# tuffy/libdvd-audio

Measured on AMD Instinct MI355X. Metric: decoded PCM Msamples/s (bit-exact) on 6ch/96k/24b MLP, higher is better.
Workload: dtype int32 (int64 accumulate)

## Files before the change

### libdvd-audio_amd/csrc/mlp_ctx.h

```cpp
#pragma once
#include <vector>

#include "hip_ws.h"
#include "mlp_decode.h"
#include "mlp_conceal.h"
#include "mlp_index.h"

using namespace mlp;

constexpr uint32_t EV_RING = 256;
constexpr uint32_t SEQ_ROUND = 1024;

struct DecodeSettings {
    uint32_t lanes_per_seg = 0;
    uint32_t pcm_layout = DVDA_PCM_PLANAR;
    uint32_t chain_form = 0;
    const int32_t *d_init_fir = nullptr;
};

struct ConcealInfo {
    uint32_t valid, status;
    uint64_t rows, frames;
};

struct ConcealState {
    bool on = false;
    dvda_mlp_hip_ctx *child = nullptr;
    DevBuf<ConcealPlan> d_plan;
    DevBuf<uint8_t> d_bytes;
    DevBuf<uint64_t> d_tab;
    DevBuf<int32_t> d_scr[CONCEAL_ROUNDS];
    DevBuf<ConcealOp> d_ops;
    DevBuf<int32_t> d_fir;
    std::vector<std::vector<dvda_mlp_conceal_span>> spans;
    std::vector<ConcealInfo> info;

    ~ConcealState() { dvda_mlp_hip_destroy(child); }
};

struct PresentState {
    uint32_t mode = DVDA_PRESENT_FULL;
    dvda_mlp_hip_ctx *child = nullptr;
    DevBuf<uint8_t> d_bytes;
    uint64_t bound = 0;
    DevBuf<uint32_t> d_info;
    DevBuf<uint32_t> d_size;
    DevBuf<uint32_t> d_sbase;
    DevBuf<uint32_t> d_len;
    DevBuf<uint32_t> d_base;
    DevBuf<uint64_t> d_off64, d_len64;
    Event ev[2];
    bool ev_set = false;
    bool map_valid = false;
    uint32_t h_nseg = 0;
    std::vector<SegRec> h_seg;
    std::vector<uint32_t> h_sbase, h_base, h_info;
    std::vector<StreamRec> h_streams;

    ~PresentState() { dvda_mlp_hip_destroy(child); }
};

struct dvda_mlp_hip_ctx {
    int device;
    uint32_t coop_min_seg;
    uint32_t max_streams, max_segments;
    DevBuf<uint8_t> d_masks;
    DevBuf<uint16_t> d_parts;
    DevBuf<uint32_t> d_tile_count;
    DevBuf<uint32_t> d_tile_base;
    DevBuf<uint64_t> d_cand_off;
    DevBuf<SegRec> d_seg;
    DevBuf<uint32_t> d_seg_frames;
    DevBuf<uint32_t> d_seg_fbase;
    DevBuf<uint32_t> d_seg_status;
    DevBuf<uint32_t> d_seg_rows;
    DevBuf<StreamRec> d_streams;
    uint32_t *d_n_cand;
    DevBuf<uint32_t> d_scan_tmp;
    DevBuf<int32_t> d_iir;
    DevBuf<uint32_t> d_mat;
    DevBuf<unsigned long long> d_dbg;
    DevBuf<int32_t> d_fir;
    DevBuf<uint32_t> d_seg_meta;
    DevBuf<uint32_t> d_yield;
    DevBuf<uint32_t> d_seg_check;
    DevBuf<uint32_t> d_cls;
    DevBuf<uint32_t> d_shape_key;
    DevBuf<uint64_t> d_soff, d_slen;
    DevBuf<uint32_t> d_rank;
    DevBuf<uint32_t> d_sorted_cnt;
    DevBuf<uint32_t> d_sorted_base;
    DevBuf<uint32_t> d_lane_seg;
    DevBuf<DecodeSummary> d_summary;
    DecodeSummary *h_summary;
    Stream st_aux;
    Event ev_fork, ev_join;
    DevBuf<uint32_t> d_seq_list;
    DevBuf<uint4> d_plan;
    DevBuf<uint4> d_scan4_tmp;
    DevBuf<uint32_t> d_def_list;
    DevBuf<uint32_t> d_head_list;
    DevBuf<uint32_t> d_chain_order;
    DevBuf<uint32_t> d_chain_hist;
    DevBuf<int32_t> d_fb;
    uint32_t rsv_segs;
    DevBuf<int32_t> d_res;
    DevBuf<uint32_t> d_brec;
    DevBuf<uint32_t> d_frec;
    uint32_t iir_lanes;
    DevBuf<dvda_pcm_crc_desc> d_crc_desc;
    DevBuf<uint32_t> d_crc_out;
    DevBuf<uint64_t> d_crc_bytes;
    DevBuf<uint32_t> d_crc_work;
    DecodeSettings set;
    const uint8_t *d_bytes;
    uint64_t total_bytes;
    const uint64_t *d_stream_off;
    const uint64_t *d_stream_len;
    uint32_t n_streams;
    uint64_t tiles;
    bool indexed;
    bool small_input;
    bool decoded;
    GraphExec idx_graph;
    const void *idx_key[4];
    uint64_t idx_key_bytes;
    uint32_t idx_key_streams;
    int idx_graph_state;
    Event ev[2 * EV_RING];
    Event ev_end[EV_RING];
    uint64_t ev_count;
    ConcealState cc;
    PresentState pp;

    uint32_t fb_slots() const { return (uint32_t)(d_fb.cap / FB_WORDS); }
    ~dvda_mlp_hip_ctx() { (void)hipHostFree(h_summary); }
};

static WsCaps ws_caps(const dvda_mlp_hip_ctx *c)
{
    WsCaps w;
    w.res = c->d_res.cap;
    w.brec = c->d_brec.cap;
    w.frec = c->d_frec.cap;
    w.fb = c->d_fb.cap;
    w.max_seg = c->max_segments;
    w.max_streams = c->max_streams;
    w.lanes = c->iir_lanes;
    w.pad = 0;
    return w;
}

static inline dvda_mlp_hip_ctx *pp_inner(const dvda_mlp_hip_ctx *c)
{
    return c && c->pp.mode == DVDA_PRESENT_SUBSTREAM0 ? c->pp.child : nullptr;
}

static inline void fill_sync_fields(dvda_mlp_stream_info &o, uint32_t sync)
{
    o.assignment = (sync >> 16) & 0x1F;
    o.substreams = (sync >> 24) & 0xF;
    o.group0_bps = sync & 0xF;
    o.group1_bps = (sync >> 4) & 0xF;
    o.group0_rate = (sync >> 8) & 0xF;
    o.group1_rate = (sync >> 12) & 0xF;
}

static void enqueue_exscan(hipStream_t st, const uint32_t *in, uint32_t *out, uint32_t *tmp, uint32_t n_host,
                           const uint32_t *n_ptr, uint32_t n_cap)
{
    const uint32_t n_max = n_ptr ? n_cap : n_host;
    if (n_max <= 4096) {
        hipLaunchKernelGGL(k_exscan_u32, dim3(1), dim3(1024), 0, st, in, out, n_host, n_ptr, n_cap);
        return;
    }
    const uint32_t blocks = (n_max + 1023) / 1024;
    hipLaunchKernelGGL(k_scan_blocks, dim3(blocks), dim3(1024), 0, st, in, out, tmp, n_host, n_ptr, n_cap);
    hipLaunchKernelGGL(k_exscan_u32, dim3(1), dim3(1024), 0, st, tmp, tmp, blocks, (const uint32_t *)nullptr, blocks);
    hipLaunchKernelGGL(k_scan_add, dim3(blocks), dim3(1024), 0, st, out, tmp, blocks, n_host, n_ptr, n_cap);
}
```

### libdvd-audio_amd/csrc/mlp_hip.hip

```cpp
#include <hip/hip_runtime.h>
#include <math.h>
#include <stdint.h>
#include <stdio.h>
#include <stdlib.h>
#include <string.h>
#include <new>
#include <vector>

#include "../../include/dvda_mlp_hip.h"
#include "mlp_step.h"
#include "mlp_decode.h"
#include "mlp_chain.h"
#include "mlp_chain_small.h"
#include "mlp_check.h"
#include "mlp_coop.h"
#include "mlp_index.h"
#include "mlp_conceal.h"
#include "mlp_present.h"
#include "pcm_unswizzle.h"
#include "wav_pack.h"
#include "pcm_digest.h"

#include "mlp_ctx.h"
#include "mlp_conceal_run.h"
#include "mlp_present_run.h"
#include "mlp_stepper.h"
#include "mlp_tiers.h"
#include "pcm_digest_run.h"

extern "C" int dvda_mlp_hip_bounds_violations(unsigned long long *out4)
{
    if (!out4)
        return DVDA_HIP_EINVAL;
    out4[0] = out4[1] = out4[2] = out4[3] = 0;
#if defined(DVDA_BOUNDS)
    HIP_TRY(hipDeviceSynchronize());
    HIP_TRY(hipMemcpyFromSymbol(out4, HIP_SYMBOL(mlp::g_bounds), 4 * sizeof(unsigned long long)));
    return 1;
#else
    return DVDA_HIP_OK;
#endif
}

extern "C" const char *dvda_mlp_hip_version(void) { return "dvda-mlp-hip 0.1 (gfx950)"; }

extern "C" int dvda_mlp_hip_create(dvda_mlp_hip_ctx **out, int device, uint32_t max_streams,
                                   uint32_t max_segments)
{
    if (!out || max_streams == 0 || max_segments == 0)
        return DVDA_HIP_EINVAL;
    int ndev = 0;
    if (hipGetDeviceCount(&ndev) != hipSuccess || ndev <= 0 || device < 0 || device >= ndev) {
        fprintf(stderr, "dvda_mlp_hip: no usable HIP device (count=%d, requested=%d)\n", ndev, device);
        return DVDA_HIP_ENODEV;
    }
    HIP_TRY(hipSetDevice(device));
    dvda_mlp_hip_ctx *c = new (std::nothrow) dvda_mlp_hip_ctx();
    if (!c)
        return DVDA_HIP_ENOMEM;
    c->device = device;
    {
        int cus = 0;
        if (hipDeviceGetAttribute(&cus, hipDeviceAttributeMultiprocessorCount, device) != hipSuccess || cus <= 0)
            cus = 256;
        c->coop_min_seg = (uint32_t)cus * 4u * 64u * 7u / 4u;
        if (const char *e = getenv("DVDA_COOP_MIN_SEG"))
            c->coop_min_seg = (uint32_t)strtoul(e, nullptr, 10);
    }
    c->max_streams = max_streams;
    c->max_segments = max_segments;
    c->idx_graph_state = getenv("DVDA_INDEX_GRAPH") && atoi(getenv("DVDA_INDEX_GRAPH")) == 0 ? -1 : 0;
    const size_t ns = (size_t)max_segments, nt = (size_t)max_streams;
    c->iir_lanes = (uint32_t)(((2 * ns + DEC_THREADS - 1) / DEC_THREADS) * DEC_THREADS);
    const size_t nl = c->iir_lanes;
    hipError_t e = hipSuccess;
    auto alloc = [&](auto &buf, size_t n) {
        if (e == hipSuccess)
            e = buf.alloc(n);
    };
    alloc(c->d_cand_off, ns);
    alloc(c->d_seg, ns + 4);
    alloc(c->d_seg_frames, ns + 1);
    alloc(c->d_seg_fbase, ns + 5);
    alloc(c->d_seg_status, ns + 4);
    alloc(c->d_seg_rows, ns);
    alloc(c->d_streams, nt);
    alloc(c->d_iir, nl * MAXCH * 16);
    alloc(c->d_mat, nl * MAXMAT * 5);
    alloc(c->d_dbg, 32);
    alloc(c->d_fir, nl * 6 * 8);
    alloc(c->d_seg_meta, nl + 4);
    alloc(c->d_yield, ns);
    alloc(c->d_seg_check, 2 * ns);
    alloc(c->d_cls, 4);
    alloc(c->d_shape_key, nt);
    alloc(c->d_soff, nt);
    alloc(c->d_slen, nt);
    alloc(c->d_rank, nt);
    alloc(c->d_sorted_cnt, nt + 1);
    alloc(c->d_sorted_base, nt + 1);
    alloc(c->d_lane_seg, ns);
    alloc(c->d_summary, 1 + SUMMARY_PARTS);
    alloc(c->d_seq_list, nt);
    alloc(c->d_plan, ns + 5);
    alloc(c->d_scan4_tmp, ns / 1024 + 4);
    alloc(c->d_def_list, ns);
    alloc(c->d_head_list, ns);
    alloc(c->d_chain_order, ns);
    alloc(c->d_chain_hist, 2 * CHAIN_BUCKETS);
    if (e == hipSuccess)
        e = hipHostMalloc((void **)&c->h_summary, sizeof(DecodeSummary), hipHostMallocDefault);
    if (e == hipSuccess)
        e = hipStreamCreateWithFlags(c->st_aux.put(), hipStreamNonBlocking);
    if (e == hipSuccess)
        e = hipEventCreateWithFlags(c->ev_fork.put(), hipEventDisableTiming);
    if (e == hipSuccess)
        e = hipEventCreateWithFlags(c->ev_join.put(), hipEventDisableTiming);
    if (e == hipSuccess)
        e = hipMemset(c->d_dbg, 0, 32 * sizeof(unsigned long long));
    if (e == hipSuccess)
        e = hipMemset(c->d_seg_meta, 0, nl * sizeof(uint32_t));
    for (uint32_t i = 0; e == hipSuccess && i < 2 * EV_RING; i++)
        e = hipEventCreate(c->ev[i].put());
    for (uint32_t i = 0; e == hipSuccess && i < EV_RING; i++)
        e = hipEventCreate(c->ev_end[i].put());
    if (e != hipSuccess) {
        fprintf(stderr, "dvda_mlp_hip: workspace allocation failed: %s\n", hipGetErrorString(e));
        delete c;
        return DVDA_HIP_ENOMEM;
    }
    *out = c;
    return DVDA_HIP_OK;
}

extern "C" void dvda_mlp_hip_destroy(dvda_mlp_hip_ctx *c)
{
    if (!c)
        return;
    (void)hipSetDevice(c->device);
#if defined(DVDA_BOUNDS)
    if (getenv("DVDA_BOUNDS_REPORT")) {
        unsigned long long v[4] = {0, 0, 0, 0};
        (void)dvda_mlp_hip_bounds_violations(v);
        fprintf(stderr, "dvda_mlp_hip: bounds violations: %llu", v[0]);
        if (v[0])
            fprintf(stderr, " (first: tag %llu index %llu capacity %llu)", v[1], v[2], v[3]);
        fprintf(stderr, "\n");
    }
#endif
    delete c;
}

static int ensure_byte_ws(dvda_mlp_hip_ctx *c, uint64_t total_bytes)
{
    const uint64_t chunks = (total_bytes + 15) / 16 + 4;
    const uint64_t tiles = (chunks + IDX_TILE_CHUNKS - 1) / IDX_TILE_CHUNKS;
    auto grow_pair = [](auto &a, uint64_t na, auto &b, uint64_t nb) {
        if (na <= a.cap)
            return DVDA_HIP_OK;
        a.release();
        b.release();
        if (a.alloc(na) == hipSuccess && b.alloc(nb) == hipSuccess)
            return DVDA_HIP_OK;
        a.release();
        return DVDA_HIP_ENOMEM;
    };
    int rc = grow_pair(c->d_masks, chunks, c->d_parts, chunks + 72);
    if (rc)
        return rc;
    uint64_t most = tiles > c->max_segments ? tiles : c->max_segments;
    if (c->max_streams > most)
        most = c->max_streams;
    if ((rc = c->d_scan_tmp.grow_exact((most + 1023) / 1024 + 2)) != 0)
        return rc;
    return grow_pair(c->d_tile_count, tiles + 1, c->d_tile_base, tiles + 1);
}

__global__ void k_init_streams(StreamRec *s, uint32_t n, uint32_t *seg_status, uint32_t *seg_rows, uint32_t *yield_req,
                               uint32_t *seg_meta, uint32_t n_seg, uint32_t *cls, uint32_t *summary_words)
{
    const uint32_t i = blockIdx.x * blockDim.x + threadIdx.x;
    if (i < 4)
        cls[i] = 0;
    if (i < (1 + SUMMARY_PARTS) * sizeof(DecodeSummary) / sizeof(uint32_t))
        summary_words[i] = 0;
    if (i < n_seg) {
        seg_status[i] = 0;
        seg_rows[i] = 0;
        yield_req[i] = 0;
        seg_meta[2 * (size_t)i] = seg_meta[2 * (size_t)i + 1] = 0;
    }
    if (i < n) {
        StreamRec r;
        r.first_seg = 0xFFFFFFFFu;
        r.n_seg = 0;
        r.sync = 0;
        r.status = 0;
        r.frames = 0;
        r.consumed = 0;
        r.rows = 0;
        s[i] = r;
    }
}

__global__ void k_reset_segments(uint32_t *seg_status, uint32_t *seg_rows, uint32_t *yield_req, uint32_t *seg_meta,
                                 uint32_t n_seg)
{
    const uint32_t i = blockIdx.x * blockDim.x + threadIdx.x;
    if (i < n_seg) {
        seg_status[i] = 0;
        seg_rows[i] = 0;
        yield_req[i] = 0;
        seg_meta[2 * (size_t)i] = seg_meta[2 * (size_t)i + 1] = 0;
    }
}

__device__ __forceinline__ void check_ranges_block(const uint64_t *__restrict__ off, const uint64_t *__restrict__ len,
                                                   uint32_t n, uint64_t total_bytes, uint64_t *__restrict__ soff,
                                                   uint64_t *__restrict__ slen, StreamRec *__restrict__ streams,
                                                   unsigned long long *s_max)
{
    const uint32_t per = (n + 1023u) / 1024u;
    const uint32_t lo = threadIdx.x * per, hi = lo + per < n ? lo + per : n;
    auto end_of = [&](uint32_t i) {
        const uint64_t o = off[i], l = len[i];
        return (o <= total_bytes && l <= total_bytes - o && (o & 15u) == 0) ? o + l : 0;
    };
    unsigned long long m = 0;
    for (uint32_t i = lo; i < hi; i++) {
        const unsigned long long e = end_of(i);
        m = e > m ? e : m;
    }
    s_max[threadIdx.x] = m;
    __syncthreads();
    for (uint32_t d = 1; d < 1024u; d <<= 1) {
        const unsigned long long v = threadIdx.x >= d ? s_max[threadIdx.x - d] : 0ull;
        __syncthreads();
        if (v > s_max[threadIdx.x])
            s_max[threadIdx.x] = v;
        __syncthreads();
    }
    unsigned long long run = threadIdx.x ? s_max[threadIdx.x - 1] : 0ull;
    for (uint32_t i = lo; i < hi; i++) {
        const uint64_t o = off[i], l = len[i];
        const bool ok = (o & 15u) == 0 && o <= total_bytes && l <= total_bytes - o && o >= run;
        const uint64_t so = ok ? o : run;
        soff[i] = so < total_bytes ? so : total_bytes;
        slen[i] = ok ? l : 0;
        if (!ok)
            streams[i].status = ST_ENVELOPE | (1u << 16);
        const unsigned long long e = end_of(i);
        run = e > run ? e : run;
    }
}

__global__ __launch_bounds__(1024) void k_check_ranges(const uint64_t *__restrict__ off, const uint64_t *__restrict__ len,
                                                       uint32_t n, uint64_t total_bytes, uint64_t *__restrict__ soff,
                                                       uint64_t *__restrict__ slen, StreamRec *__restrict__ streams)
{
    __shared__ unsigned long long s_max[1024];
    check_ranges_block(off, len, n, total_bytes, soff, slen, streams, s_max);
}

constexpr uint64_t SMALL_INPUT_BYTES = 4096u * 1024u;

static void enqueue_index(dvda_mlp_hip_ctx *c, hipStream_t st, const uint8_t *d_bytes, uint64_t total_bytes,
                          const uint64_t *d_stream_off, const uint64_t *d_stream_len, uint32_t n_streams)
{
    const uint64_t tiles = c->tiles;
    const uint32_t ms = c->max_segments;
    {
        uint32_t n_init = n_streams > ms ? n_streams : ms;
        if (n_init < 1024)
            n_init = 1024;
        hipLaunchKernelGGL(k_init_streams, dim3((n_init + 255) / 256), dim3(256), 0, st, c->d_streams,
                           n_streams, c->d_seg_status, c->d_seg_rows, c->d_yield, c->d_seg_meta, ms, c->d_cls,
                           reinterpret_cast<uint32_t *>(c->d_summary.p));
        hipLaunchKernelGGL(k_check_ranges, dim3(1), dim3(1024), 0, st, d_stream_off, d_stream_len, n_streams, total_bytes,
                           c->d_soff, c->d_slen, c->d_streams);
        d_stream_off = c->d_soff;
        d_stream_len = c->d_slen;
    }
    hipLaunchKernelGGL(k_sync_mask, dim3((unsigned)tiles), dim3(IDX_THREADS), 0, st, d_bytes,
                       total_bytes, c->d_masks, c->d_tile_count, c->d_parts);
    enqueue_exscan(st, c->d_tile_count, c->d_tile_base, c->d_scan_tmp, (uint32_t)tiles, nullptr, (uint32_t)tiles);
    hipLaunchKernelGGL(k_sync_scatter, dim3((unsigned)tiles), dim3(IDX_THREADS), 0, st, c->d_masks,
                       total_bytes, c->d_tile_base, c->d_cand_off, ms);
    hipLaunchKernelGGL(k_chase, dim3((ms + 255) / 256), dim3(256), 0, st, d_bytes, d_stream_off,
                       d_stream_len, n_streams, c->d_cand_off, c->d_n_cand, ms, c->d_seg,
                       c->d_seg_frames, c->d_streams, c->d_cls);
    hipLaunchKernelGGL(k_mark_dead, dim3((ms + 255) / 256), dim3(256), 0, st, d_stream_off, d_stream_len,
                       c->d_n_cand, ms, c->d_seg, c->d_seg_frames, c->d_streams);
    enqueue_exscan(st, c->d_seg_frames, c->d_seg_fbase, c->d_scan_tmp, 0u, c->d_n_cand, ms);
    const bool pack = !(total_bytes <= SMALL_INPUT_BYTES);
    hipLaunchKernelGGL(k_link, dim3((ms + 255) / 256), dim3(256), 0, st, d_stream_off, d_stream_len,
                       c->d_n_cand, ms, c->d_seg, c->d_seg_fbase, c->d_streams, n_streams, c->d_shape_key,
                       c->d_cls + (pack ? 2 : 3));
    hipStream_t sp = st;
    bool forked = false;
    if (pack && st != nullptr && c->st_aux && hipEventRecord(c->ev_fork, st) == hipSuccess &&
        hipStreamWaitEvent(c->st_aux, c->ev_fork, 0) == hipSuccess) {
        sp = c->st_aux;
        forked = true;
    }
    if (pack) {
    hipLaunchKernelGGL(k_stream_rank, dim3((n_streams + 255) / 256), dim3(256), 0, sp, c->d_shape_key, c->d_streams,
                       n_streams, c->d_rank, c->d_sorted_cnt, c->d_cls + 2);
    enqueue_exscan(sp, c->d_sorted_cnt, c->d_sorted_base, c->d_scan_tmp, n_streams, nullptr, n_streams);
    (void)hipMemsetAsync(c->d_lane_seg, 0xFF, (size_t)ms * sizeof(uint32_t), sp);
    hipLaunchKernelGGL(k_lane_perm, dim3((ms + 255) / 256), dim3(256), 0, sp, c->d_seg, c->d_streams, c->d_n_cand, ms,
                       c->d_rank, c->d_sorted_base, c->d_cls + 2, c->d_lane_seg);
    }
    hipLaunchKernelGGL(k_au_check, dim3((unsigned)(((uint64_t)ms * CHK_GROUP + CHK_THREADS - 1) / CHK_THREADS)),
                       dim3(CHK_THREADS), 0, st, d_bytes, c->d_parts, c->d_seg, c->d_n_cand, ms, c->d_streams, c->d_seg_check);
    if (forked) {
        (void)hipEventRecord(c->ev_join, sp);
        (void)hipStreamWaitEvent(st, c->ev_join, 0);
    }
}

static int index_source(dvda_mlp_hip_ctx *c, const uint8_t *d_bytes, uint64_t total_bytes,
                        const uint64_t *d_stream_off, const uint64_t *d_stream_len, uint32_t n_streams, void *stream_)
{
    if (!c || !d_bytes || !d_stream_off || !d_stream_len || n_streams == 0 || total_bytes == 0)
        return DVDA_HIP_EINVAL;
    if (n_streams > c->max_streams)
        return DVDA_HIP_ECAPACITY;
    if (((uintptr_t)d_bytes & 15) != 0)
        return DVDA_HIP_EINVAL;
    hipStream_t st = (hipStream_t)stream_;
    HIP_TRY(hipSetDevice(c->device));
    c->cc.spans.clear();
    c->cc.info.clear();
    int rc = ensure_byte_ws(c, total_bytes);
    if (rc)
        return rc;
    c->d_bytes = d_bytes;
    c->total_bytes = total_bytes;
    c->d_stream_off = d_stream_off;
    c->d_stream_len = d_stream_len;
    c->n_streams = n_streams;
    const uint64_t chunks = (total_bytes + 15) / 16;
    const uint64_t tiles = (chunks + IDX_TILE_CHUNKS - 1) / IDX_TILE_CHUNKS;
    c->tiles = tiles;
    c->d_n_cand = c->d_tile_base + tiles;

    c->small_input = total_bytes <= SMALL_INPUT_BYTES;
    const bool same = c->idx_graph_state > 0 && c->idx_key[0] == d_bytes && c->idx_key[1] == d_stream_off &&
                      c->idx_key[2] == d_stream_len && c->idx_key[3] == (const void *)st &&
                      c->idx_key_bytes == total_bytes && c->idx_key_streams == n_streams;
    if (c->idx_graph_state == 2 && same) {
        if (hipGraphLaunch(c->idx_graph, st) == hipSuccess) {
            c->indexed = true;
            c->decoded = false;
            return DVDA_HIP_OK;
        }
        (void)hipGetLastError();
        c->idx_graph_state = -1;
    } else if (c->idx_graph_state == 1 && same && st != nullptr) {
        hipGraph_t g = nullptr;
        bool ok = hipStreamBeginCapture(st, hipStreamCaptureModeThreadLocal) == hipSuccess;
        if (ok) {
            enqueue_index(c, st, d_bytes, total_bytes, d_stream_off, d_stream_len, n_streams);
            ok = hipStreamEndCapture(st, &g) == hipSuccess && g != nullptr;
        }
        if (ok) {
            ok = hipGraphInstantiate(c->idx_graph.put(), g, nullptr, nullptr, 0) == hipSuccess;
        }
        if (g)
            (void)hipGraphDestroy(g);
        if (ok && hipGraphLaunch(c->idx_graph, st) == hipSuccess) {
            c->idx_graph_state = 2;
            c->indexed = true;
            c->decoded = false;
            return DVDA_HIP_OK;
        }
        (void)hipGetLastError();
        c->idx_graph_state = -1;
    } else if (c->idx_graph_state >= 0) {
        c->idx_key[0] = d_bytes;
        c->idx_key[1] = d_stream_off;
        c->idx_key[2] = d_stream_len;
        c->idx_key[3] = (const void *)st;
        c->idx_key_bytes = total_bytes;
        c->idx_key_streams = n_streams;
        c->idx_graph_state = 1;
    }
    enqueue_index(c, st, d_bytes, total_bytes, d_stream_off, d_stream_len, n_streams);
    HIP_TRY(hipGetLastError());
    c->indexed = true;
    c->decoded = false;
    return DVDA_HIP_OK;
}

extern "C" int dvda_mlp_hip_index(dvda_mlp_hip_ctx *c, const uint8_t *d_bytes, uint64_t total_bytes,
                                  const uint64_t *d_stream_off, const uint64_t *d_stream_len,
                                  uint32_t n_streams, void *stream_)
{
    const int rc = index_source(c, d_bytes, total_bytes, d_stream_off, d_stream_len, n_streams, stream_);
    if (rc != DVDA_HIP_OK || c->pp.mode != DVDA_PRESENT_SUBSTREAM0)
        return rc;
    return present_index(c, (hipStream_t)stream_);
}

static int read_summary(dvda_mlp_hip_ctx *c, hipStream_t st)
{
    HIP_TRY(hipMemcpyAsync(c->h_summary, c->d_summary, sizeof(DecodeSummary), hipMemcpyDeviceToHost, st));
    HIP_TRY(hipStreamSynchronize(st));
    return DVDA_HIP_OK;
}

__global__ void k_chain_guard(uint4 *plan, const uint32_t *n_seg_ptr, uint32_t max_seg, WsCaps caps, uint32_t seg_cap)
{
    uint32_t n = *n_seg_ptr;
    if (n > max_seg)
        n = max_seg;
    const uint4 t = plan[n];
    const unsigned long long rows = t.x, segs = t.y;
    const ChainNeed need = chain_need(rows, segs);
    if (segs > seg_cap || need.res > caps.res || need.brec > caps.brec || need.frec > caps.frec)
        plan[n] = make_uint4(t.x, 0, 0, 0);
}

static int grow_chain_ws(dvda_mlp_hip_ctx *c, uint64_t rows, uint64_t segs)
{
    const ChainNeed need = chain_need(rows, segs);
    int rc;
    if ((rc = c->d_res.grow(need.res)) != 0 || (rc = c->d_brec.grow(need.brec)) != 0)
        return rc;
    return c->d_frec.grow(need.frec);
}

static int grow_fb(dvda_mlp_hip_ctx *c, uint32_t round)
{
    return c->d_fb.grow_exact((uint64_t)round * FB_WORDS);
}

static dvda_mlp_hip_ctx *pp_forward(dvda_mlp_hip_ctx *c)
{
    dvda_mlp_hip_ctx *x = pp_inner(c);
    if (x)
        x->set = c->set;
    return x;
}

extern "C" int dvda_mlp_hip_reserve(dvda_mlp_hip_ctx *c, uint64_t chain_pcm_frames, uint32_t chain_segments,
                                    uint32_t seq_streams)
{
    if (!c)
        return DVDA_HIP_EINVAL;
    if (dvda_mlp_hip_ctx *x = pp_forward(c))
        return dvda_mlp_hip_reserve(x, chain_pcm_frames, chain_segments, seq_streams);
    HIP_TRY(hipSetDevice(c->device));
    if (chain_pcm_frames >> 32)
        return DVDA_HIP_ECAPACITY;
    if (chain_segments || chain_pcm_frames) {
        const int rc = grow_chain_ws(c, chain_pcm_frames, chain_segments);
        if (rc)
            return rc;
        if (chain_segments > c->rsv_segs)
            c->rsv_segs = chain_segments;
    }
    return grow_fb(c, seq_streams < SEQ_ROUND ? seq_streams : SEQ_ROUND);
}

struct KernelChoice {
    bool coop_only, lanes_only;
    uint32_t force;

    explicit KernelChoice(const dvda_mlp_hip_ctx *c)
        : coop_only(c->set.lanes_per_seg == 64 || (c->set.lanes_per_seg == 0 && c->small_input)),
          lanes_only(c->set.lanes_per_seg == 3), force((coop_only || lanes_only) ? 0u : c->set.lanes_per_seg)
    {
    }
};

struct PassWork {
    uint32_t segs;
    uint64_t rows;
    uint32_t max_rows;
    bool few;
    uint32_t n_seq;
};
static PassWork pass_work(const dvda_mlp_hip_ctx *c, bool blocking)
{
    const DecodeSummary &s = *c->h_summary;
    if (blocking)
        return {s.chain_segs, s.chain_rows, s.chain_max_rows, s.waiting <= CHAIN_SMALL_STREAMS, s.seq_streams};
    return {c->rsv_segs, 0, 0, c->rsv_segs <= CHAIN_SMALL_SEGS, c->fb_slots()};
}

static DecodeArgs decode_args(const dvda_mlp_hip_ctx *c, const KernelChoice &k, int32_t *d_pcm, const uint64_t *d_out_off,
                              const uint64_t *d_out_stride)
{
    DecodeArgs a;
    memset(&a, 0, sizeof(a));
    a.bytes = c->d_bytes;
    a.total_bytes = c->total_bytes;
// ... 489 lines not shown
```

### libdvd-audio_amd/csrc/mlp_index.h

```cpp
#pragma once
#include <hip/hip_runtime.h>
#include <stdint.h>
#include "mlp_tables.h"

namespace mlp {

struct SegRec {
    uint64_t off;
    uint64_t end;
    uint32_t stream;
    uint32_t nframes;
    uint32_t flags;
    uint32_t sync;
    uint32_t ndrop;
    uint32_t prev;
};
constexpr uint32_t SYNC_PARAMS = 0x00FFFFFFu;
constexpr uint32_t MAX_DROP = 64;

struct StreamRec {
    uint32_t first_seg;
    uint32_t n_seg;
    uint32_t sync;
    uint32_t status;
    uint64_t frames;
    uint64_t consumed;
    uint64_t rows;
};

constexpr int IDX_THREADS = 256;
constexpr int IDX_CHUNKS_PER_THREAD = 16;
constexpr int IDX_TILE_CHUNKS = IDX_THREADS * IDX_CHUNKS_PER_THREAD;

__device__ __forceinline__ uint32_t ld_u8(const uint8_t *p, uint64_t i) { return p[i]; }

__device__ __forceinline__ bool sync_frame_at(const uint8_t *b, uint64_t p, uint64_t limit)
{
    if (p + 32 > limit)
        return false;
    const uint32_t size = 2u * (((ld_u8(b, p) & 0x0Fu) << 8) | ld_u8(b, p + 1));
    if (size < 32)
        return false;
    if (ld_u8(b, p + 4) != 0xF8 || ld_u8(b, p + 5) != 0x72 || ld_u8(b, p + 6) != 0x6F ||
        ld_u8(b, p + 7) != 0xBB)
        return false;
    const uint32_t count = ld_u8(b, p + 20) >> 4;
    return count == 1 || count == 2;
}

__device__ __forceinline__ uint64_t ld_hdr8(const uint8_t *b, uint64_t p)
{
    const uint16_t *h = reinterpret_cast<const uint16_t *>(b + p);
    return (uint64_t)h[0] | ((uint64_t)h[1] << 16) | ((uint64_t)h[2] << 32) | ((uint64_t)h[3] << 48);
}

__device__ __forceinline__ bool sync_frame_hdr(const uint8_t *b, uint64_t p, uint64_t limit, uint64_t hdr)
{
    if (p + 32 > limit)
        return false;
    const uint32_t size = 2u * ((((uint32_t)hdr & 0x0Fu) << 8) | (((uint32_t)hdr >> 8) & 0xFFu));
    if (size < 32 || (uint32_t)(hdr >> 32) != 0xBB6F72F8u)
        return false;
    const uint32_t count = ld_u8(b, p + 20) >> 4;
    return count == 1 || count == 2;
}

__device__ __forceinline__ uint32_t packed_sync_at(const uint8_t *b, uint64_t p)
{
    return (ld_u8(b, p + 8) >> 4) | ((ld_u8(b, p + 8) & 0xFu) << 4) | ((ld_u8(b, p + 9) >> 4) << 8) |
           ((ld_u8(b, p + 9) & 0xFu) << 12) | ((ld_u8(b, p + 11) & 0x1Fu) << 16) | ((ld_u8(b, p + 20) >> 4) << 24);
}

__device__ const CheckTables d_chk = make_check();

__device__ __forceinline__ uint32_t mask_chunk(const uint8_t *__restrict__ bytes, uint64_t total_bytes, uint64_t chunk,
                                               const uint8_t *s_slice, uint32_t &part)
{
    const uint4 *q = reinterpret_cast<const uint4 *>(bytes) + chunk;
    const uint4 a = q[0], c = q[1];
    uint32_t w[8] = {a.x, a.y, a.z, a.w, c.x, c.y, c.z, c.w};
    uint32_t m = 0;
    uint32_t any = 0;
#pragma unroll
    for (int k = 1; k <= 4; k++) {
        const uint32_t y = w[k] ^ 0x72F872F8u;
        any |= (y - 0x00010001u) & ~y & 0x80008000u;
    }
    if (__builtin_expect(any != 0, 0)) {
#pragma unroll
        for (int j = 0; j < 8; j++) {
            const int h = j + 2;
            const uint32_t lo = (h & 1) ? (w[h >> 1] >> 16) : (w[h >> 1] & 0xFFFFu);
            const uint32_t hi = ((h + 1) & 1) ? (w[(h + 1) >> 1] >> 16) : (w[(h + 1) >> 1] & 0xFFFFu);
            if (lo == 0x72F8u && hi == 0xBB6Fu) {
                if (sync_frame_at(bytes, chunk * 16 + 2 * j, total_bytes))
                    m |= 1u << j;
            }
        }
    }
    uint32_t c0 = 0;
#pragma unroll
    for (int k = 0; k < 4; k++)
        c0 ^= s_slice[(15 - 4 * k) * 256 + (w[k] & 0xFFu)] ^ s_slice[(14 - 4 * k) * 256 + ((w[k] >> 8) & 0xFFu)] ^
              s_slice[(13 - 4 * k) * 256 + ((w[k] >> 16) & 0xFFu)] ^ s_slice[(12 - 4 * k) * 256 + (w[k] >> 24)];
    uint32_t px = w[0] ^ w[1] ^ w[2] ^ w[3];
    px ^= px >> 16;
    px = (px ^ (px >> 8)) & 0xFFu;
    part = c0 | (px << 8);
    return m;
}

__global__ __launch_bounds__(IDX_THREADS) void k_sync_mask(const uint8_t *__restrict__ bytes,
                                                           uint64_t total_bytes,
                                                           uint8_t *__restrict__ masks,
                                                           uint32_t *__restrict__ tile_count,
                                                           uint16_t *__restrict__ parts)
{
    __shared__ uint32_t s_cnt[IDX_THREADS / 64];
    __shared__ uint8_t s_slice[16 * 256];
    for (int i = threadIdx.x; i < 16 * 256 / 16; i += IDX_THREADS)
        reinterpret_cast<uint4 *>(s_slice)[i] = reinterpret_cast<const uint4 *>(d_chk.slice)[i];
    __syncthreads();
    const uint64_t n_chunks = (total_bytes + 15) >> 4;
    const uint64_t tile0 = (uint64_t)blockIdx.x * IDX_TILE_CHUNKS;
    uint32_t cnt = 0;
    for (int k = 0; k < IDX_CHUNKS_PER_THREAD; k++) {
        const uint64_t chunk = tile0 + (uint64_t)k * IDX_THREADS + threadIdx.x;
        if (chunk >= n_chunks)
            break;
        uint32_t part;
        const uint32_t m = mask_chunk(bytes, total_bytes, chunk, s_slice, part);
        masks[chunk] = (uint8_t)m;
        cnt += __popc(m);
        parts[chunk] = (uint16_t)part;
    }
    for (int o = 32; o > 0; o >>= 1)
        cnt += __shfl_down(cnt, o, 64);
    if ((threadIdx.x & 63) == 0)
        s_cnt[threadIdx.x >> 6] = cnt;
    __syncthreads();
    if (threadIdx.x == 0) {
        uint32_t t = 0;
        for (int i = 0; i < IDX_THREADS / 64; i++)
            t += s_cnt[i];
        tile_count[blockIdx.x] = t;
    }
}

__global__ __launch_bounds__(1024) void k_exscan_u32(const uint32_t *__restrict__ in,
                                                     uint32_t *__restrict__ out, uint32_t n_host,
                                                     const uint32_t *__restrict__ n_ptr,
                                                     uint32_t n_cap)
{
    __shared__ uint32_t s_part[1024];
    uint32_t n = n_ptr ? *n_ptr : n_host;
    if (n > n_cap)
        n = n_cap;
    const uint32_t per = (n + 1023) / 1024;
    const uint32_t lo = threadIdx.x * per;
    const uint32_t hi = lo + per < n ? lo + per : n;
    uint32_t sum = 0;
    for (uint32_t i = lo; i < hi; i++)
        sum += in[i];
    s_part[threadIdx.x] = sum;
    __syncthreads();
    for (int o = 1; o < 1024; o <<= 1) {
        uint32_t v = threadIdx.x >= (uint32_t)o ? s_part[threadIdx.x - o] : 0;
        __syncthreads();
        s_part[threadIdx.x] += v;
        __syncthreads();
    }
    uint32_t run = threadIdx.x ? s_part[threadIdx.x - 1] : 0;
    for (uint32_t i = lo; i < hi; i++) {
        const uint32_t v = in[i];
        out[i] = run;
        run += v;
    }
    if (threadIdx.x == 1023)
        out[n] = s_part[1023];
}

__global__ __launch_bounds__(1024) void k_scan_blocks(const uint32_t *__restrict__ in,
                                                      uint32_t *__restrict__ out,
                                                      uint32_t *__restrict__ block_sum, uint32_t n_host,
                                                      const uint32_t *__restrict__ n_ptr, uint32_t n_cap)
{
    __shared__ uint32_t s_v[1024];
    uint32_t n = n_ptr ? *n_ptr : n_host;
    if (n > n_cap)
        n = n_cap;
    const uint32_t i = blockIdx.x * 1024 + threadIdx.x;
    const uint32_t v = i < n ? in[i] : 0;
    s_v[threadIdx.x] = v;
    __syncthreads();
    for (int o = 1; o < 1024; o <<= 1) {
        const uint32_t t = threadIdx.x >= (uint32_t)o ? s_v[threadIdx.x - o] : 0;
        __syncthreads();
        s_v[threadIdx.x] += t;
        __syncthreads();
    }
    if (i < n)
        out[i] = s_v[threadIdx.x] - v;
    if (threadIdx.x == 1023)
        block_sum[blockIdx.x] = s_v[1023];
}

__global__ __launch_bounds__(1024) void k_scan_add(uint32_t *__restrict__ out,
                                                   const uint32_t *__restrict__ block_base,
                                                   uint32_t n_blocks, uint32_t n_host,
                                                   const uint32_t *__restrict__ n_ptr, uint32_t n_cap)
{
    uint32_t n = n_ptr ? *n_ptr : n_host;
    if (n > n_cap)
        n = n_cap;
    const uint32_t i = blockIdx.x * 1024 + threadIdx.x;
    if (i < n)
        out[i] += block_base[blockIdx.x];
    if (i == 0)
        out[n] = block_base[n_blocks];
}

__global__ __launch_bounds__(IDX_THREADS) void k_sync_scatter(const uint8_t *__restrict__ masks,
                                                              uint64_t total_bytes,
                                                              const uint32_t *__restrict__ tile_base,
                                                              uint64_t *__restrict__ cand_off,
                                                              uint32_t max_cand)
{
    __shared__ uint32_t s_wave[IDX_THREADS / 64];
    const uint64_t n_chunks = (total_bytes + 15) >> 4;
    const uint64_t first = (uint64_t)blockIdx.x * IDX_TILE_CHUNKS +
                           (uint64_t)threadIdx.x * IDX_CHUNKS_PER_THREAD;
    static_assert(IDX_CHUNKS_PER_THREAD == 16, "one 16-byte load of mask bytes per thread");
    uint8_t m[IDX_CHUNKS_PER_THREAD];
    uint32_t cnt = 0;
    if (first + IDX_CHUNKS_PER_THREAD <= n_chunks) {
        const uint4 q = *reinterpret_cast<const uint4 *>(masks + first);
        const uint32_t w[4] = {q.x, q.y, q.z, q.w};
#pragma unroll
        for (int k = 0; k < IDX_CHUNKS_PER_THREAD; k++)
            m[k] = (uint8_t)(w[k >> 2] >> (8 * (k & 3)));
        cnt = __popc(q.x) + __popc(q.y) + __popc(q.z) + __popc(q.w);
    } else {
#pragma unroll
        for (int k = 0; k < IDX_CHUNKS_PER_THREAD; k++) {
            m[k] = (first + k < n_chunks) ? masks[first + k] : 0;
            cnt += __popc((uint32_t)m[k]);
        }
    }
    uint32_t inc = cnt;
#pragma unroll
    for (int o = 1; o < 64; o <<= 1) {
        const uint32_t v = __shfl_up(inc, o, 64);
        if ((int)(threadIdx.x & 63) >= o)
            inc += v;
    }
    if ((threadIdx.x & 63) == 63)
        s_wave[threadIdx.x >> 6] = inc;
    __syncthreads();
    uint32_t before = 0;
    for (uint32_t w = 0; w < (threadIdx.x >> 6); w++)
        before += s_wave[w];
    uint32_t at = tile_base[blockIdx.x] + before + inc - cnt;
    if (cnt == 0)
        return;
#pragma unroll
    for (int k = 0; k < IDX_CHUNKS_PER_THREAD; k++) {
        uint32_t mk = m[k];
        while (mk) {
            const int j = __ffs(mk) - 1;
            mk &= mk - 1;
            if (at < max_cand)
                cand_off[at] = (first + k) * 16 + 2 * j;
            at++;
        }
    }
}

__device__ __forceinline__ uint32_t find_stream(const uint64_t *__restrict__ stream_off,
                                                uint32_t n_streams, uint64_t p)
{
    uint32_t lo = 0, hi = n_streams;
    while (hi - lo > 1) {
        const uint32_t mid = (lo + hi) >> 1;
        if (stream_off[mid] <= p)
            lo = mid;
        else
            hi = mid;
    }
    return lo;
}

constexpr uint32_t SEG_DEAD = 1u << 24;

__device__ __forceinline__ void chase_one(uint32_t i, const uint8_t *__restrict__ bytes,
                                          const uint64_t *__restrict__ stream_off,
                                          const uint64_t *__restrict__ stream_len, uint32_t n_streams,
                                          const uint64_t *__restrict__ cand_off, SegRec *__restrict__ seg,
                                          uint32_t *__restrict__ seg_frames, StreamRec *__restrict__ streams,
                                          uint32_t *__restrict__ cls)
{
    const uint64_t off = cand_off[i];
    const uint32_t s = find_stream(stream_off, n_streams, off);
    const uint64_t s_begin = stream_off[s];
    const uint64_t s_end = s_begin + stream_len[s];
    SegRec r;
    r.off = off;
    r.stream = s;
    r.flags = 0;
    r.nframes = 0;
    r.sync = 0;
    r.ndrop = 0;
    r.prev = 0xFFFFFFFFu;
    uint64_t p = off;
    const bool outside = off >= s_end;
    if (outside) {
        r.flags = SEG_DEAD;
        r.end = off;
    } else if ((off - s_begin) & 1) {
        r.flags = 1u << 16;
        r.end = off;
    } else if (!sync_frame_at(bytes, off, s_end)) {
        r.flags = SEG_DEAD;
        r.end = off;
    } else {
        r.sync = packed_sync_at(bytes, off);
        const bool own = sync_frame_at(bytes, s_begin, s_end) &&
                         ((packed_sync_at(bytes, s_begin) ^ r.sync) & SYNC_PARAMS) == 0;
        uint32_t n = 0;
        uint64_t hdr = ld_hdr8(bytes, p);
        for (;;) {
            if (p + 4 > s_end) {
                if (p != s_end)
                    r.flags |= 1u << 21;
                break;
            }
            const uint32_t size = 2u * ((((uint32_t)hdr & 0x0Fu) << 8) | (((uint32_t)hdr >> 8) & 0xFFu));
            if (size < 4) {
                r.flags |= 1u << 4;
                break;
            }
            if (p + size > s_end) {
                r.flags |= 1u << 21;
                break;
            }
            p += size;
            n++;
            hdr = ld_hdr8(bytes, p);
            if (sync_frame_hdr(bytes, p, s_end, hdr)) {
                if (((packed_sync_at(bytes, p) ^ r.sync) & SYNC_PARAMS) == 0 || (!own && r.ndrop >= MAX_DROP))
                    break;
                r.ndrop++;
            }
        }
        r.nframes = n;
        r.end = p;
    }
    seg[i] = r;
    seg_frames[i] = r.nframes - r.ndrop;
    bool first = (i == 0);
    if (!first) {
        const uint64_t prev = cand_off[i - 1];
        first = prev < s_begin;
    }
    if (first && !outside) {
        streams[s].first_seg = i;
        streams[s].sync = r.sync;
        const uint32_t S = (r.sync >> 24) & 0xFu;
        if (S == 1 || S == 2)
            cls[S - 1] = 1u;
    }
}

__global__ __launch_bounds__(256) void k_chase(const uint8_t *__restrict__ bytes,
                                               const uint64_t *__restrict__ stream_off,
                                               const uint64_t *__restrict__ stream_len,
                                               uint32_t n_streams,
                                               const uint64_t *__restrict__ cand_off,
                                               const uint32_t *__restrict__ n_cand_ptr,
                                               uint32_t max_cand, SegRec *__restrict__ seg,
                                               uint32_t *__restrict__ seg_frames,
                                               StreamRec *__restrict__ streams, uint32_t *__restrict__ cls)
{
    const uint32_t i = blockIdx.x * blockDim.x + threadIdx.x;
    uint32_t n_cand = *n_cand_ptr;
    if (n_cand > max_cand)
        n_cand = max_cand;
    if (i >= n_cand)
        return;
    chase_one(i, bytes, stream_off, stream_len, n_streams, cand_off, seg, seg_frames, streams, cls);
}


constexpr uint32_t STEP_CAP = 4096;
__device__ __forceinline__ void mark_dead_one(uint32_t i, uint32_t n_cand, const uint64_t *__restrict__ stream_off,
                                              const uint64_t *__restrict__ stream_len, SegRec *__restrict__ seg,
                                              uint32_t *__restrict__ seg_frames, const StreamRec *__restrict__ streams)
{
    if (i >= n_cand || i == 0)
        return;
    const uint32_t s = seg[i].stream;
    const uint64_t off = seg[i].off;
    if (seg[i - 1].stream != s)
        return;
    const uint32_t want = streams[s].sync & SYNC_PARAMS;
    const bool foreign = (seg[i].sync & SYNC_PARAMS) != want;
    uint32_t steps = 0;
    if (!foreign) {
        uint32_t seen = 0;
        for (uint32_t q = i; q-- > 0 && seen <= MAX_DROP + 1 && seg[q].stream == s;) {
            if (++steps > STEP_CAP) {
                seg[i].flags |= 1u << 16;
                return;
            }
            if ((seg[q].sync & SYNC_PARAMS) != want)
                continue;
            seen++;
            if (seg[q].end == off)
                return;
        }
    }
    const uint64_t s_end = stream_off[s] + stream_len[s];
    uint32_t seen_b = 0;
    for (uint32_t q = i; q-- > 0 && seen_b <= MAX_DROP + 1 && seg[q].stream == s;) {
        const uint64_t e = seg[q].end;
        if (++steps > STEP_CAP) {
            seg[i].flags |= 1u << 16;
// ... 191 lines not shown
```

Baseline: 262,600.

## Stage per-tile sync candidates in mask kernel and replace scan+scatter with bucket gather

The sync-mask kernel now builds a sorted list of up to 64 candidate offsets per tile in shared memory and writes it to a compact staging buffer. It writes the full mask bytes only for tiles that overflow that cap, and it adds each tile's count atomically into a per-256-tile bucket. A new gather kernel derives global offsets from the bucket sums plus an in-block scan and emits the candidates, falling back to reading masks for dense tiles. This removes the multi-kernel exclusive scan and the full mask write and re-read, at the cost of shared-memory atomics, a quadratic rank step per tile and a serial bucket prefix sum in each gather block.

After: 261,400. About the same (-0.4%).

```diff
diff --git a/libdvd-audio_amd/csrc/mlp_ctx.h b/libdvd-audio_amd/csrc/mlp_ctx.h
--- a/libdvd-audio_amd/csrc/mlp_ctx.h
+++ b/libdvd-audio_amd/csrc/mlp_ctx.h
@@ -67,7 +67,8 @@
     DevBuf<uint8_t> d_masks;
     DevBuf<uint16_t> d_parts;
     DevBuf<uint32_t> d_tile_count;
-    DevBuf<uint32_t> d_tile_base;
+    DevBuf<uint16_t> d_cand_stage;
+    DevBuf<uint32_t> d_bucket;
     DevBuf<uint64_t> d_cand_off;
     DevBuf<SegRec> d_seg;
     DevBuf<uint32_t> d_seg_frames;
diff --git a/libdvd-audio_amd/csrc/mlp_hip.hip b/libdvd-audio_amd/csrc/mlp_hip.hip
--- a/libdvd-audio_amd/csrc/mlp_hip.hip
+++ b/libdvd-audio_amd/csrc/mlp_hip.hip
@@ -165,21 +165,24 @@
         a.release();
         return DVDA_HIP_ENOMEM;
     };
-    int rc = grow_pair(c->d_masks, chunks, c->d_parts, chunks + 72);
+    int rc = grow_pair(c->d_masks, tiles * IDX_TILE_CHUNKS, c->d_parts, chunks + 72);
     if (rc)
         return rc;
-    uint64_t most = tiles > c->max_segments ? tiles : c->max_segments;
-    if (c->max_streams > most)
-        most = c->max_streams;
+    const uint64_t most = c->max_streams > c->max_segments ? c->max_streams : c->max_segments;
     if ((rc = c->d_scan_tmp.grow_exact((most + 1023) / 1024 + 2)) != 0)
         return rc;
-    return grow_pair(c->d_tile_count, tiles + 1, c->d_tile_base, tiles + 1);
+    if ((rc = c->d_bucket.grow_exact(tiles / IDX_BUCKET_TILES + 2)) != 0)
+        return rc;
+    return grow_pair(c->d_tile_count, tiles + 1, c->d_cand_stage, tiles * TILE_CAND_CAP);
 }
 
 __global__ void k_init_streams(StreamRec *s, uint32_t n, uint32_t *seg_status, uint32_t *seg_rows, uint32_t *yield_req,
-                               uint32_t *seg_meta, uint32_t n_seg, uint32_t *cls, uint32_t *summary_words)
+                               uint32_t *seg_meta, uint32_t n_seg, uint32_t *cls, uint32_t *summary_words,
+                               uint32_t *bucket, uint32_t n_bucket)
 {
     const uint32_t i = blockIdx.x * blockDim.x + threadIdx.x;
+    if (i < n_bucket)
+        bucket[i] = 0;
     if (i < 4)
         cls[i] = 0;
     if (i < (1 + SUMMARY_PARTS) * sizeof(DecodeSummary) / sizeof(uint32_t))
@@ -269,23 +272,25 @@
 {
     const uint64_t tiles = c->tiles;
     const uint32_t ms = c->max_segments;
+    const uint32_t n_bucket = (uint32_t)((tiles + IDX_BUCKET_TILES - 1) / IDX_BUCKET_TILES);
     {
         uint32_t n_init = n_streams > ms ? n_streams : ms;
         if (n_init < 1024)
             n_init = 1024;
+        if (n_init < n_bucket)
+            n_init = n_bucket;
         hipLaunchKernelGGL(k_init_streams, dim3((n_init + 255) / 256), dim3(256), 0, st, c->d_streams,
                            n_streams, c->d_seg_status, c->d_seg_rows, c->d_yield, c->d_seg_meta, ms, c->d_cls,
-                           reinterpret_cast<uint32_t *>(c->d_summary.p));
+                           reinterpret_cast<uint32_t *>(c->d_summary.p), c->d_bucket.p, n_bucket);
         hipLaunchKernelGGL(k_check_ranges, dim3(1), dim3(1024), 0, st, d_stream_off, d_stream_len, n_streams, total_bytes,
                            c->d_soff, c->d_slen, c->d_streams);
         d_stream_off = c->d_soff;
         d_stream_len = c->d_slen;
     }
     hipLaunchKernelGGL(k_sync_mask, dim3((unsigned)tiles), dim3(IDX_THREADS), 0, st, d_bytes,
-                       total_bytes, c->d_masks, c->d_tile_count, c->d_parts);
-    enqueue_exscan(st, c->d_tile_count, c->d_tile_base, c->d_scan_tmp, (uint32_t)tiles, nullptr, (uint32_t)tiles);
-    hipLaunchKernelGGL(k_sync_scatter, dim3((unsigned)tiles), dim3(IDX_THREADS), 0, st, c->d_masks,
-                       total_bytes, c->d_tile_base, c->d_cand_off, ms);
+                       total_bytes, c->d_masks, c->d_tile_count, c->d_parts, c->d_cand_stage, c->d_bucket);
+    hipLaunchKernelGGL(k_sync_gather, dim3(n_bucket), dim3(IDX_THREADS), 0, st, c->d_masks, c->d_tile_count,
+                       c->d_bucket, (uint32_t)tiles, c->d_cand_stage, c->d_cand_off, ms, c->d_n_cand);
     hipLaunchKernelGGL(k_chase, dim3((ms + 255) / 256), dim3(256), 0, st, d_bytes, d_stream_off,
                        d_stream_len, n_streams, c->d_cand_off, c->d_n_cand, ms, c->d_seg,
                        c->d_seg_frames, c->d_streams, c->d_cls);
@@ -343,7 +348,7 @@
     const uint64_t chunks = (total_bytes + 15) / 16;
     const uint64_t tiles = (chunks + IDX_TILE_CHUNKS - 1) / IDX_TILE_CHUNKS;
     c->tiles = tiles;
-    c->d_n_cand = c->d_tile_base + tiles;
+    c->d_n_cand = c->d_bucket + (tiles + IDX_BUCKET_TILES - 1) / IDX_BUCKET_TILES;
 
     c->small_input = total_bytes <= SMALL_INPUT_BYTES;
     const bool same = c->idx_graph_state > 0 && c->idx_key[0] == d_bytes && c->idx_key[1] == d_stream_off &&
diff --git a/libdvd-audio_amd/csrc/mlp_index.h b/libdvd-audio_amd/csrc/mlp_index.h
--- a/libdvd-audio_amd/csrc/mlp_index.h
+++ b/libdvd-audio_amd/csrc/mlp_index.h
@@ -110,40 +110,113 @@
     return m;
 }
 
+constexpr uint32_t TILE_CAND_CAP = 64;
+constexpr uint32_t IDX_BUCKET_TILES = 256;
+
+__device__ __forceinline__ uint32_t tile_rank(uint32_t cnt, uint32_t *s_wave, uint32_t &total)
+{
+    uint32_t inc = cnt;
+#pragma unroll
+    for (int o = 1; o < 64; o <<= 1) {
+        const uint32_t v = __shfl_up(inc, o, 64);
+        if ((int)(threadIdx.x & 63) >= o)
+            inc += v;
+    }
+    if ((threadIdx.x & 63) == 63)
+        s_wave[threadIdx.x >> 6] = inc;
+    __syncthreads();
+    uint32_t before = 0, all = 0;
+#pragma unroll
+    for (uint32_t w = 0; w < IDX_THREADS / 64; w++) {
+        const uint32_t v = s_wave[w];
+        before += w < (threadIdx.x >> 6) ? v : 0u;
+        all += v;
+    }
+    total = all;
+    return before + inc - cnt;
+}
+
+template <typename F>
+__device__ __forceinline__ void tile_emit(const uint4 &q, uint32_t first, uint32_t at, F emit)
+{
+    const uint32_t w[4] = {q.x, q.y, q.z, q.w};
+#pragma unroll
+    for (int k = 0; k < IDX_CHUNKS_PER_THREAD; k++) {
+        uint32_t mk = (w[k >> 2] >> (8 * (k & 3))) & 0xFFu;
+        while (mk) {
+            const int j = __ffs(mk) - 1;
+            mk &= mk - 1;
+            emit(at, (first + k) * 16u + 2u * j);
+            at++;
+        }
+    }
+}
+
 __global__ __launch_bounds__(IDX_THREADS) void k_sync_mask(const uint8_t *__restrict__ bytes,
                                                            uint64_t total_bytes,
                                                            uint8_t *__restrict__ masks,
                                                            uint32_t *__restrict__ tile_count,
-                                                           uint16_t *__restrict__ parts)
-{
-    __shared__ uint32_t s_cnt[IDX_THREADS / 64];
+                                                           uint16_t *__restrict__ parts,
+                                                           uint16_t *__restrict__ stage,
+                                                           uint32_t *__restrict__ bucket)
+{
+    static_assert(IDX_CHUNKS_PER_THREAD == 16, "one 16-byte store of mask bytes per thread");
+    static_assert(TILE_CAND_CAP <= 64, "the list is ranked by the lanes of one wave");
+    __shared__ uint32_t s_n;
+    __shared__ uint16_t s_list[TILE_CAND_CAP];
     __shared__ uint8_t s_slice[16 * 256];
+    __shared__ __attribute__((aligned(16))) uint8_t s_mask[IDX_TILE_CHUNKS];
     for (int i = threadIdx.x; i < 16 * 256 / 16; i += IDX_THREADS)
         reinterpret_cast<uint4 *>(s_slice)[i] = reinterpret_cast<const uint4 *>(d_chk.slice)[i];
+    reinterpret_cast<uint4 *>(s_mask)[threadIdx.x] = make_uint4(0, 0, 0, 0);
+    if (threadIdx.x == 0)
+        s_n = 0;
     __syncthreads();
     const uint64_t n_chunks = (total_bytes + 15) >> 4;
     const uint64_t tile0 = (uint64_t)blockIdx.x * IDX_TILE_CHUNKS;
-    uint32_t cnt = 0;
+    uint32_t mw[IDX_CHUNKS_PER_THREAD / 4] = {0, 0, 0, 0};
+#pragma unroll
     for (int k = 0; k < IDX_CHUNKS_PER_THREAD; k++) {
         const uint64_t chunk = tile0 + (uint64_t)k * IDX_THREADS + threadIdx.x;
         if (chunk >= n_chunks)
             break;
         uint32_t part;
         const uint32_t m = mask_chunk(bytes, total_bytes, chunk, s_slice, part);
-        masks[chunk] = (uint8_t)m;
-        cnt += __popc(m);
+        mw[k >> 2] |= m << (8 * (k & 3));
         parts[chunk] = (uint16_t)part;
     }
-    for (int o = 32; o > 0; o >>= 1)
-        cnt += __shfl_down(cnt, o, 64);
-    if ((threadIdx.x & 63) == 0)
-        s_cnt[threadIdx.x >> 6] = cnt;
+    if (__builtin_expect((mw[0] | mw[1] | mw[2] | mw[3]) != 0, 0)) {
+#pragma unroll
+        for (int k = 0; k < IDX_CHUNKS_PER_THREAD; k++) {
+            uint32_t mk = (mw[k >> 2] >> (8 * (k & 3))) & 0xFFu;
+            if (!mk)
+                continue;
+            const uint32_t in_tile = k * IDX_THREADS + threadIdx.x;
+            s_mask[in_tile] = (uint8_t)mk;
+            while (mk) {
+                const int j = __ffs(mk) - 1;
+                mk &= mk - 1;
+                const uint32_t at = atomicAdd(&s_n, 1u);
+                if (at < TILE_CAND_CAP)
+                    s_list[at] = (uint16_t)(in_tile * 16u + 2u * j);
+            }
+        }
+    }
     __syncthreads();
+    const uint32_t total = s_n;
+    if (total > TILE_CAND_CAP) {
+        reinterpret_cast<uint4 *>(masks + tile0)[threadIdx.x] = reinterpret_cast<const uint4 *>(s_mask)[threadIdx.x];
+    } else if (threadIdx.x < total) {
+        const uint32_t mine = s_list[threadIdx.x];
+        uint32_t rank = 0;
+        for (uint32_t j = 0; j < total; j++)
+            rank += s_list[j] < mine ? 1u : 0u;
+        stage[(uint64_t)blockIdx.x * TILE_CAND_CAP + rank] = (uint16_t)mine;
+    }
     if (threadIdx.x == 0) {
-        uint32_t t = 0;
-        for (int i = 0; i < IDX_THREADS / 64; i++)
-            t += s_cnt[i];
-        tile_count[blockIdx.x] = t;
+        tile_count[blockIdx.x] = total;
+        if (total)
+            atomicAdd(&bucket[blockIdx.x / IDX_BUCKET_TILES], total);
     }
 }
 
@@ -220,58 +293,77 @@
         out[n] = block_base[n_blocks];
 }
 
-__global__ __launch_bounds__(IDX_THREADS) void k_sync_scatter(const uint8_t *__restrict__ masks,
-                                                              uint64_t total_bytes,
-                                                              const uint32_t *__restrict__ tile_base,
-                                                              uint64_t *__restrict__ cand_off,
-                                                              uint32_t max_cand)
-{
+__global__ __launch_bounds__(IDX_THREADS) void k_sync_gather(const uint8_t *__restrict__ masks,
+                                                             const uint32_t *__restrict__ tile_count,
+                                                             const uint32_t *bucket, uint32_t n_tiles,
+                                                             const uint16_t *__restrict__ stage,
+                                                             uint64_t *__restrict__ cand_off, uint32_t max_cand,
+                                                             uint32_t *n_cand_out)
+{
+    static_assert(IDX_BUCKET_TILES == IDX_THREADS, "a thread per tile of the bucket");
+    static_assert(TILE_CAND_CAP % 8 == 0, "a staging row is read 8 entries at a time");
     __shared__ uint32_t s_wave[IDX_THREADS / 64];
-    const uint64_t n_chunks = (total_bytes + 15) >> 4;
-    const uint64_t first = (uint64_t)blockIdx.x * IDX_TILE_CHUNKS +
-                           (uint64_t)threadIdx.x * IDX_CHUNKS_PER_THREAD;
-    static_assert(IDX_CHUNKS_PER_THREAD == 16, "one 16-byte load of mask bytes per thread");
-    uint8_t m[IDX_CHUNKS_PER_THREAD];
-    uint32_t cnt = 0;
-    if (first + IDX_CHUNKS_PER_THREAD <= n_chunks) {
-        const uint4 q = *reinterpret_cast<const uint4 *>(masks + first);
-        const uint32_t w[4] = {q.x, q.y, q.z, q.w};
-#pragma unroll
-        for (int k = 0; k < IDX_CHUNKS_PER_THREAD; k++)
-            m[k] = (uint8_t)(w[k >> 2] >> (8 * (k & 3)));
-        cnt = __popc(q.x) + __popc(q.y) + __popc(q.z) + __popc(q.w);
+    __shared__ uint32_t s_sum[IDX_THREADS / 64];
+    __shared__ unsigned long long s_fallback[IDX_THREADS / 64];
+    __shared__ uint32_t s_base[IDX_THREADS];
+    const uint32_t tile = blockIdx.x * IDX_BUCKET_TILES + threadIdx.x;
+    const uint32_t cnt = tile < n_tiles ? tile_count[tile] : 0u;
+    const uint32_t n_sum = blockIdx.x == 0 ? (n_tiles + IDX_BUCKET_TILES - 1) / IDX_BUCKET_TILES : blockIdx.x;
+    uint32_t sum = 0;
+    for (uint32_t i = threadIdx.x; i < n_sum; i += IDX_THREADS)
+        sum += bucket[i];
+    for (int o = 32; o > 0; o >>= 1)
+        sum += __shfl_xor(sum, o, 64);
+    if ((threadIdx.x & 63) == 0)
+        s_sum[threadIdx.x >> 6] = sum;
+    const unsigned long long fb = __ballot(cnt > TILE_CAND_CAP);
+    if ((threadIdx.x & 63) == 0)
+        s_fallback[threadIdx.x >> 6] = fb;
+    uint32_t all;
+    uint32_t base = tile_rank(cnt, s_wave, all);
+    sum = 0;
+#pragma unroll
+    for (int w = 0; w < IDX_THREADS / 64; w++)
+        sum += s_sum[w];
+    if (blockIdx.x == 0) {
+        if (threadIdx.x == 0)
+            *n_cand_out = sum;
     } else {
-#pragma unroll
-        for (int k = 0; k < IDX_CHUNKS_PER_THREAD; k++) {
-            m[k] = (first + k < n_chunks) ? masks[first + k] : 0;
-            cnt += __popc((uint32_t)m[k]);
-        }
-    }
-    uint32_t inc = cnt;
-#pragma unroll
-    for (int o = 1; o < 64; o <<= 1) {
-        const uint32_t v = __shfl_up(inc, o, 64);
-        if ((int)(threadIdx.x & 63) >= o)
-            inc += v;
-    }
-    if ((threadIdx.x & 63) == 63)
-        s_wave[threadIdx.x >> 6] = inc;
-    __syncthreads();
-    uint32_t before = 0;
-    for (uint32_t w = 0; w < (threadIdx.x >> 6); w++)
-        before += s_wave[w];
-    uint32_t at = tile_base[blockIdx.x] + before + inc - cnt;
-    if (cnt == 0)
-        return;
-#pragma unroll
-    for (int k = 0; k < IDX_CHUNKS_PER_THREAD; k++) {
-        uint32_t mk = m[k];
-        while (mk) {
-            const int j = __ffs(mk) - 1;
-            mk &= mk - 1;
-            if (at < max_cand)
-                cand_off[at] = (first + k) * 16 + 2 * j;
-            at++;
+        base += sum;
+    }
+    s_base[threadIdx.x] = base;
+    const uint64_t tile_bytes = (uint64_t)IDX_TILE_CHUNKS * 16;
+    if (cnt && cnt <= TILE_CAND_CAP) {
+        const uint4 *row = reinterpret_cast<const uint4 *>(stage + (uint64_t)tile * TILE_CAND_CAP);
+        const uint64_t off0 = tile * tile_bytes;
+        for (uint32_t i = 0; i < cnt; i += 8) {
+            const uint4 q = row[i >> 3];
+            const uint32_t w[4] = {q.x, q.y, q.z, q.w};
+#pragma unroll
+            for (uint32_t e = 0; e < 8; e++) {
+                const uint32_t at = base + i + e;
+                if (i + e < cnt && at < max_cand)
+                    cand_off[at] = off0 + ((w[e >> 1] >> (16 * (e & 1))) & 0xFFFFu);
+            }
+        }
+    }
+    for (uint32_t w = 0; w < IDX_THREADS / 64; w++) {
+        __syncthreads();
+        unsigned long long left = s_fallback[w];
+        while (left) {
+            const uint32_t t = w * 64 + (uint32_t)__ffsll(left) - 1;
+            left &= left - 1;
+            const uint32_t ft = blockIdx.x * IDX_BUCKET_TILES + t;
+            const uint4 q = reinterpret_cast<const uint4 *>(masks + (uint64_t)ft * IDX_TILE_CHUNKS)[threadIdx.x];
+            const uint32_t c = __popc(q.x) + __popc(q.y) + __popc(q.z) + __popc(q.w);
+            uint32_t tile_all;
+            const uint32_t at = s_base[t] + tile_rank(c, s_wave, tile_all);
+            const uint64_t off0 = ft * tile_bytes;
+            tile_emit(q, threadIdx.x * IDX_CHUNKS_PER_THREAD, at, [&](uint32_t r, uint32_t o) {
+                if (r < max_cand)
+                    cand_off[r] = off0 + o;
+            });
+            __syncthreads();
         }
     }
 }
```
